# denyingmxd/CFPNet

Measured on AMD Instinct MI355X. Metric: depth maps/sec @ 480x640 bf16 (whole job; per_gpu = value / n_gpus); abs_rel vs CPU oracle, higher is better.
Workload: dtype bf16; 1 GPU; batch=8 480x640 RGB + 8x8-zone ToF, eval forward incl. the prob output [B,256,H/2,W/2] written in the storage dtype (bf16: 2 bytes/element); layers=hist2image combine1 image x2 (CFPNet), parallelism=single GPU

## Files before the change

### cfpnet_amd/csrc/conv_route.hip

```cpp
#include "conv_route.h"

namespace {

int tile_count(int variant, int M, int Cout) {
  static const int bm[4] = {256, 256, 128, 128}, bn[4] = {16, 32, 64, 128};
  return cdiv(M, bm[variant]) * cdiv(Cout, bn[variant]);
}

int pick_splits(int variant, int M, int Cout, int K, int dtype) {
  const int bk = is16(dtype) ? 32 : 16;
  const int nk = cdiv(K, bk);
  const int tiles = tile_count(variant, M, Cout);
  if (tiles >= 128 || nk < 16) return 1;
  int s = cdiv(256, tiles);
  if (s > nk / 6) s = nk / 6;
  if (s > 32) s = 32;
  return s < 2 ? 1 : s;
}

}

static int g_force_variant = -1, g_force_splits = -1;
int g_use_v1 = 0;
int g_tput = 0;
int g_probe = 0;
int g_x3_ad = 0;
int g_x3_small_m = 4800, g_x3_small_k = 1 << 30;
int g_x3_occ = 1;
static int x3_occ_of(int v) { return v == 13 ? 34 : v == 16 ? 35 : v == 15 ? 36 : v; }
static int x3_ad_of(int v) { return v == 26 ? 28 : v == 14 ? 29 : v == 13 ? 30 : v == 23 ? 31 : v == 16 ? 32 : v; }
int g_small_s2 = 1;
int g_up_halo = 1;
int g_halo_s2 = 1;
int g_halo = 1;
extern int g_bin_head_x3_rows;
int g_x3_ln_fused = 1;
int g_halo_x3 = 1;
static bool halo_x3_wins(long long M, int Cin, int Cout, bool tput) { return M >= (tput ? 30000 : 15000) && Cin <= 56; }
static int chunk_x3_variant(long long M, int Cin, int Cout, bool tput) {
  if (Cin % 32 != 0) return -1;
  if (Cin == 32) {
    if (Cout <= 32) return M >= 30000 ? 45 : -1;
    if (Cout > 64 && Cout <= 128 && !tput) return (M >= 30000 && M < 200000) ? 44 : -1;
    return -1;
  }
  if (Cout > 128) return (tput && M >= 9000) ? 36 : -1;
  if (Cout > 64) return M >= 30000 ? ((!tput && M < 200000) ? 44 : 36) : -1;
  if (Cout <= 32) return M >= (tput ? 30000 : 15000) ? 45 : -1;
  if (M >= 100000) return 38;
  if (M >= 30000) return tput ? 38 : 24;
  return -1;
}
int g_chunk16 = 1;
static int chunk16_variant(long long M, int Cin, int Cout, bool tput) {
  if (Cin <= 64 || Cin % 8 != 0 || Cout <= 0 || Cout % 8 != 0 || M <= 0 || g_chunk16 == 0) return -1;
  if (g_chunk16 == 2) return Cout > 64 ? 0 : 1;
  if (M >= 30000 && M < 200000) return 1;
  if (M >= 8000 && M < 12000) return (Cout > 128) != tput ? 1 : -1;
  return -1;
}
extern "C" int cfp_conv3x3_chunk_variant(int M, int Cin, int Cout, int in_flight) { return chunk16_variant(M, Cin, Cout, in_flight > 1); }
static bool halo_wins_s2(long long M, int Cout) { return g_halo == 2 || (g_halo == 1 && g_halo_s2 && M >= 30000 && Cout <= 160); }
static bool halo_wins(long long M, int Cout, bool tput) {
  if (g_halo == 2) return true;
  if (g_halo == 1 && tput && M >= 100000 && Cout <= 64) return true;
  return g_halo == 1 && ((M >= 300000 && (Cout <= 32 || Cout == 128)) || (M >= 100000 && Cout > 128 && Cout <= 160) ||
                         (M >= 30000 && Cout > 160 && Cout <= 256));
}
void cfp_tail_x3_debug_set(int value);
void cfp_fold_debug_set(int v);
void cfp_tail16_debug_set(int value);
void cfp_attn_apply_debug_set(int value);
void cfp_dwl3_debug_set(int value);
void cfp_dwl_wgrad_debug_set(int value);
void cfp_wgrad_debug_set(int value);
void cfp_bn_debug_set(int key, int value);
void cfp_attn_debug_set(int value);
int cfp_dw_debug_set(int key, int value);
extern "C" int cfp_debug_set(int key, int value) {
  switch (key) {
    case 3: case 4: case 5: case 6: case 9: case 10: case 11: return cfp_dw_debug_set(key, value);
    case 30: cfp_dwl3_debug_set(value); return CFP_OK;
    case 32: g_x3_occ = value; return CFP_OK;
    case 33: g_x3_small_m = value; return CFP_OK;
    case 34: g_x3_small_k = value; return CFP_OK;
    case 35: cfp_tail_x3_debug_set(value); return CFP_OK;
    case 37: cfp_fold_debug_set(value); return CFP_OK;
    case 38: cfp_attn_apply_debug_set(value); return CFP_OK;
    case 39: cfp_tail16_debug_set(value); return CFP_OK;
    case 40: g_chunk16 = value; return CFP_OK;
    case 17: g_tput = value; return CFP_OK;
    case 16: g_probe = (g_probe & 16) | value; return CFP_OK;
    case 29: g_x3_ad = value; return CFP_OK;
    case 28: g_probe = (g_probe & ~16) | (value ? 16 : 0); return CFP_OK;
    case 15: g_small_s2 = value; return CFP_OK;
    case 14: g_up_halo = value; return CFP_OK;
    case 19: cfp_attn_debug_set(value); return CFP_OK;
    case 20: case 21: cfp_bn_debug_set(key, value); return CFP_OK;
    case 22: cfp_wgrad_debug_set(value); return CFP_OK;
    case 23: cfp_dwl_wgrad_debug_set(value); return CFP_OK;
    case 18: g_halo_s2 = value; return CFP_OK;
    case 12: g_halo = value; return CFP_OK;
    case 24: g_halo_x3 = value; return CFP_OK;
    case 25: g_bin_head_x3_rows = value; return CFP_OK;
    case 26: g_x3_ln_fused = value; return CFP_OK;
    case 27: conv3x3_halo_debug_odd_pitch(value); return CFP_OK;
    case 13: conv3x3_halo_debug_stages(value); return CFP_OK;
    case 0: g_force_variant = value; return CFP_OK;
    case 1: g_force_splits = value; return CFP_OK;
    case 2: g_use_v1 = value; return CFP_OK;
    default: cfp_set_error("cfp_debug_set: unknown key"); return CFP_EINVAL;
  }
}

extern "C" int cfp_conv2d_variant(int M, int Cout) {
  if (Cout <= 16) return 0;
  if (Cout <= 32) return 1;
  if (Cout <= 64) return 2;
  long long t128 = (long long)cdiv(M, 128) * cdiv(Cout, 128);
  bool waste = (Cout % 128) != 0 && (Cout % 128) <= 64;
  return (t128 < 192 || waste) ? 2 : 3;
}

namespace {

struct Plan2 { int variant, splits; bool gen1; int direct; };

Plan2 plan2(long long M, int N, int K, int rpb, int B, bool allow_split, bool conv3x3s1 = false, bool tput = false) {
  Plan2 pl{4, 1, false, -1};
  const int nv = igemm2_num_variants();
  const bool big = M >= 100000, mid = M >= 30000;
  if (N <= 16) {
    if (big && K <= 144) pl.gen1 = true; else pl.variant = 16;
  } else if (N <= 32) {
    if (conv3x3s1 && K >= 576 && mid) pl.direct = 4;
    else if ((big && K <= 128) || (mid && K <= 64)) pl.gen1 = true;
    else pl.variant = mid ? 16 : 9;
  } else if (N <= 64) {
    if ((big && K <= 160) || (mid && K <= 64)) pl.gen1 = true;
    else pl.variant = big ? 14 : mid ? 13 : 4;
  } else {
    if ((big && K <= 288) || (mid && K <= 64)) pl.gen1 = true;
    else if ((M * N >= 614400ll * 128 && K >= 512) || (mid && K >= 2048)) pl.variant = 1;
    else if (mid) pl.variant = (N % 128 != 0 && N % 128 <= 64) ? 14 : 15;
    else if ((N >= 256 && K >= 2048) || N >= 1024) pl.variant = 12;
    else if (conv3x3s1 && N <= 128 && K >= 1152 && M >= 8000) pl.direct = 4;
    else pl.variant = 4;
  }
  if (rpb > 0) { pl.gen1 = false; pl.direct = -1; if (pl.variant != 12) pl.variant = 4; }
  if (pl.variant == 4 && !pl.gen1 && pl.direct < 0 && K >= 768) {
    const long long tm = rpb > 0 ? (long long)B * ((rpb + 63) / 64) : (M + 63) / 64;
    if (tm * ((N + 63) / 64) <= 256) pl.variant = 19;
  }
  if (allow_split && K >= 2048 && (M <= 1100 || ((M + 63) / 64) * ((N + 63) / 64) <= 48)) { pl.variant = 4; pl.splits = 8; pl.gen1 = false; pl.direct = -1; }
  if (pl.variant == 4 && pl.splits == 1 && !pl.gen1 && pl.direct < 0 && g_small_s2) pl.variant = 13;
  if (pl.variant == 12 && pl.splits == 1 && !pl.gen1 && pl.direct < 0 && g_small_s2) pl.variant = 15;
  if (pl.variant == 13 && !pl.gen1 && pl.direct < 0 && rpb == 0 && M >= 9000 && M < 30000 && N >= 512 && K <= 256 && g_small_s2) pl.variant = 14;
  if (!tput && !g_tput && conv3x3s1 && rpb == 0 && !pl.gen1 && pl.splits == 1 && pl.direct < 0 && M <= 2400 && N >= 256 && K >= 2048) pl.direct = 4;
  if ((tput || g_tput) && !pl.gen1 && pl.splits == 1) {
    if (pl.direct < 0 && M <= 20000 && N >= 256 && K >= 2048) pl.variant = 1;
    if (pl.direct < 0 && pl.variant == 13 && rpb == 0 && M >= 30000 && M < 100000 && N <= 64 && K >= 512) pl.variant = 14;
  }
  if (g_force_variant >= 200 && conv3x3s1 && g_force_variant - 200 < conv3x3_num_variants()) { pl.direct = g_force_variant - 200; pl.gen1 = false; pl.splits = 1; }
  else if (g_force_variant >= 0) pl.direct = -1;
  if (g_force_variant >= 0 && g_force_variant < nv) { pl.variant = g_force_variant; pl.gen1 = false; }
  if (g_force_splits >= 1) pl.splits = g_force_splits;
  if (pl.splits > 1 && pl.variant >= 19 && pl.variant <= 21 && g_force_variant < 0) pl.variant = 4;
  if (pl.direct >= 0) { pl.gen1 = false; pl.splits = 1; }
  return pl;
}

int pick_ln_variant(int Cout, long long M) {
  switch (Cout) {
    case 128: return M <= 20000 ? 12 : 1;
    case 64: return 2;
    case 32: return 8;
    case 16: return 11;
    default: return -1;
  }
}

}

static Plan2 plan_x3(long long M, int N, int K, int rpb, int B, bool allow_split, bool tput, bool piw_split = true) {
  Plan2 pl = plan2(M, N, 2 * (cdiv(K, 32) * 32), rpb, B, allow_split, false, tput);
  if (pl.gen1 || pl.direct >= 0) pl.variant = N <= 16 ? 10 : N <= 32 ? 16 : N <= 64 ? 14 : K <= 64 ? 16 : 1;
  pl.gen1 = false; pl.direct = -1;
  if (pl.variant == 0 || pl.variant == 1) pl.variant = 26;
  if (tput && pl.variant == 15 && M >= 9000 && N >= 128 && N <= 256 && K >= 500) pl.variant = 26;
  if (pl.variant < 0 || pl.variant >= igemm_x3_num_variants()) pl.variant = 13;
  if (!tput && rpb == 0 && pl.splits <= 1 && M <= 2400 && K >= 2000 && N >= 128 && (pl.variant == 15 || pl.variant == 13)) pl.variant = 19;
  if (!tput && rpb == 0 && allow_split && pl.splits <= 1 && K >= 2000 && (M <= 1200 || (M <= 4800 && K >= 2500))) {
    pl.variant = 13; pl.splits = (M <= 1200 && K >= 3000) ? 8 : 4;
  }
  if (!tput && rpb == 0 && pl.splits <= 1 && M <= 512 && N >= 512 && K <= 512) pl.variant = 17;
  if (!tput && pl.splits <= 1 && pl.variant == 13 && M <= g_x3_small_m && K <= g_x3_small_k) pl.variant = 17;
  if (!tput && rpb == 0 && pl.splits >= 4 && M <= 160 && (pl.variant == 4 || pl.variant == 13)) pl.variant = 17;
  if (rpb > 0 && !tput && piw_split && pl.splits <= 1) {
    const long long tiles = (long long)B * cdiv(rpb, 64) * cdiv(N, 64);
    const int nks = cdiv(K, 32);
    if (tiles <= 64 && nks >= 20) { pl.variant = 4; pl.splits = nks >= 40 ? 8 : 4; }
  }
  if (g_x3_ad && pl.splits <= 1) pl.variant = x3_ad_of(pl.variant);
  if (tput && g_x3_occ && pl.splits <= 1) pl.variant = x3_occ_of(pl.variant);
  return pl;
}

static ConvRoute route_x3(const ConvP& p, const ConvArgs& a) {
  ConvRoute r{};
  const bool tput = a.in_flight || g_tput != 0;
  const int rpb = a.per_image ? p.Ho * p.Wo : 0;
  const int chunk_v = g_halo_x3 ? chunk_x3_variant(p.M, p.Cin, p.Cout, tput) : -1;
  const bool halo = !a.per_image && !a.ln && conv3x3_halo_x3_takes(p) &&
                    (g_force_variant >= 500 || (g_force_variant < 0 && g_halo_x3 && (chunk_v >= 0 || halo_x3_wins(p.M, p.Cin, p.Cout, tput))));
  auto plan = [&](bool piw_split) { return plan_x3(p.M, p.Cout, p.K, rpb, p.B, rpb == 0, tput, piw_split); };
  Plan2 pl = plan(true);
  if (g_force_variant >= 400 && g_force_variant - 400 < igemm_x3_num_variants()) pl.variant = g_force_variant - 400;
  if (g_force_splits >= 1) pl.splits = g_force_splits;
  if (pl.splits > 1 && pl.variant >= 19) pl.variant = 4;
  if (pl.splits > 1 && a.ws_bytes < (size_t)pl.splits * p.M * p.Cout * sizeof(float) + (a.want_tickets ? CFP_CONV_TICKET_BYTES : 0)) {
    if (rpb > 0) pl = plan(false);
    pl.splits = 1;
  }
  int ln_v = -1;
  if (a.ln && rpb == 0 && g_x3_ln_fused) ln_v = p.Cout == 128 ? (p.M >= 30000 ? 26 : 27) : p.Cout == 64 ? (p.M >= 100000 ? 14 : 13) : p.Cout == 32 ? 16 : p.Cout == 16 ? 11 : -1;
  const int cv4 = p.Cout / 4;
  if (a.ln && pl.splits > 1 && p.Cout % 4 == 0 && cv4 <= 64 && (cv4 & (cv4 - 1)) == 0 && g_x3_ln_fused) {
    r.ln = ConvLn::Reduce;
  } else if (ln_v >= 0) {
    pl.variant = g_x3_ad ? x3_ad_of(ln_v) : ln_v; pl.splits = 1; r.ln = ConvLn::Tile;
  } else if (a.ln) {
    r.ln = ConvLn::After;
  }
  if (a.want_tickets && pl.splits > 1 && r.ln != ConvLn::Reduce) {
    int bm, bn, st;
    igemm_x3_variant_shape(pl.variant, &bm, &bn, &st);
    const long long tiles = (rpb > 0 ? (long long)p.B * cdiv(rpb, bm) : cdiv(p.M, bm)) * cdiv(p.Cout, bn);
    r.tickets = tiles <= CFP_TICKET_SLOTS && (long long)pl.splits * p.M * p.Cout * 4 < (1ll << 31) - 16;
  }
  r.fallback = {ConvFamily::X3, pl.variant};
  r.splits = pl.splits;
  r.first = r.fallback;
  if (halo) {
// ... 111 lines not shown
```

### cfpnet_amd/csrc/head_conv0.hip

```cpp
#include "common.h"

namespace {

typedef __attribute__((address_space(3))) void* lds_ptr_t;

constexpr int HC_C = 128;
constexpr int HC_NB = 256;
constexpr int HC_CIN = 32;
constexpr int HC_K0 = 9 * HC_CIN;
constexpr int HC_K3 = 9 * HC_C;
constexpr int HC_STEPS = HC_K3 / 64;
constexpr int HC_WSTAGE = HC_C * 128;
constexpr int HC_TW = 20, HC_TPIX = HC_TW * HC_TW, HC_TP = 80;
constexpr int HC_UW = 18, HC_UPIX = HC_UW * HC_UW, HC_UP = 288;
constexpr int HC_UGROUPS = (HC_UPIX + 15) / 16;
constexpr int HC_OFF_T = 2 * HC_WSTAGE;
constexpr int HC_OFF_U = 65536;
constexpr int HC_OFF_K = HC_OFF_U + HC_UPIX * HC_UP;
constexpr int HC_LDS = HC_OFF_K + 4 * 256 * 4;
constexpr int HC_BM = 256;
constexpr int HC_PPITCH = HC_BM + 8;
constexpr unsigned HC_OOB = 0x80000000u;
static_assert(HC_OFF_T + HC_TPIX * HC_TP <= HC_OFF_U, "t halo");
static_assert(HC_NB * HC_PPITCH * 2 <= HC_OFF_K, "prob staging must end before the constants");
static_assert(HC_LDS <= 160 * 1024, "LDS of a CU");

struct HeadC0P {
  const void* t; const void* w0; const float* scale0; const float* shift0;
  const void* w3; const float* scale3; const float* shift3;
  const void* wout; const float* bias_out; const float* centers;
  void* prob; float* pred;
  int t_ld, B, H, W, HW, tiles_x, tiles_y;
  int probe;
};

__device__ __forceinline__ void hc_handover() {
  asm volatile("s_waitcnt vmcnt(0) lgkmcnt(0)" ::: "memory");
  __syncthreads();
  asm volatile("" ::: "memory");
}

template <typename H>
__global__ __launch_bounds__(512, 1) void depth_head_conv0_kernel(HeadC0P p) {
  extern __shared__ __attribute__((aligned(16))) unsigned char smem[];
  unsigned char* sT = smem + HC_OFF_T;
  unsigned char* sU = smem + HC_OFF_U;
  float* sK = reinterpret_cast<float*>(smem + HC_OFF_K);
  const int tid = threadIdx.x;
  const int lane = tid & 63;
  const int wave = __builtin_amdgcn_readfirstlane(tid >> 6);
  const int fr = lane & 15, fq = lane >> 4;
  const int rsub = lane >> 3;
  const int lc = (lane & 7) ^ rsub;
  int bid = xcd_remap(blockIdx.x, gridDim.x);
  const int x0 = (bid % p.tiles_x) * 16; bid /= p.tiles_x;
  const int y0 = (bid % p.tiles_y) * 16;
  const int b = bid / p.tiles_y;

  const int live = (p.probe & 1) ? 0 : 1;
  const auto rs_t = __builtin_amdgcn_make_buffer_rsrc((void*)p.t, 0, (int)((unsigned)p.B * (unsigned)p.HW * (unsigned)p.t_ld * 2u) * live, 0x00020000);
  const auto rs_w0 = __builtin_amdgcn_make_buffer_rsrc((void*)p.w0, 0, HC_C * HC_K0 * 2 * live, 0x00020000);
  const auto rs_w3 = __builtin_amdgcn_make_buffer_rsrc((void*)p.w3, 0, HC_C * HC_K3 * 2 * live, 0x00020000);
  const auto rs_o = __builtin_amdgcn_make_buffer_rsrc((void*)p.wout, 0, HC_NB * HC_C * 2 * live, 0x00020000);

  auto issue_w0 = [&](int ks, int buf) {
#pragma unroll
    for (int i = 0; i < 2; ++i) {
      const int g = i * 8 + wave;
      const unsigned v = (ks * 8 + lc) * 8 < HC_K0 ? (unsigned)(g * 8 + rsub) * (unsigned)(HC_K0 * 2) + (unsigned)lc * 16u : HC_OOB;
      __builtin_amdgcn_raw_ptr_buffer_load_lds(rs_w0, (lds_ptr_t)(smem + buf * HC_WSTAGE + g * 1024), 16, (int)v, ks * 128, 0, 0);
    }
  };
  auto issue_w3 = [&](int ks, int buf) {
#pragma unroll
    for (int i = 0; i < 2; ++i) {
      const int g = i * 8 + wave;
      const unsigned v = (unsigned)(g * 8 + rsub) * (unsigned)(HC_K3 * 2) + (unsigned)lc * 16u;
      __builtin_amdgcn_raw_ptr_buffer_load_lds(rs_w3, (lds_ptr_t)(smem + buf * HC_WSTAGE + g * 1024), 16, (int)v, ks * 128, 0, 0);
    }
  };
  auto issue_wout = [&](int half, int off) {
#pragma unroll
    for (int q = 0; q < 4; ++q) {
      const int g = q * 8 + wave;
      const unsigned v = (unsigned)(g * 8 + rsub) * (unsigned)(HC_C * 2) + (unsigned)lc * 16u;
      __builtin_amdgcn_raw_ptr_buffer_load_lds(rs_o, (lds_ptr_t)(smem + off + g * 1024), 16, (int)v, half * 128, 0, 0);
    }
  };

  issue_w0(0, 0);

  {
    u32x4 v[4];
    int dst[4];
#pragma unroll
    for (int n = 0; n < 4; ++n) {
      const int i = tid + n * 512;
      const int px = i >> 2, ch = i & 3;
      const int hy = px / HC_TW, hx = px - hy * HC_TW;
      const int y = y0 - 2 + hy, x = x0 - 2 + hx;
      const bool ok = px < HC_TPIX && (unsigned)y < (unsigned)p.H && (unsigned)x < (unsigned)p.W;
      const unsigned off = ok ? (unsigned)((b * p.H + y) * p.W + x) * (unsigned)p.t_ld * 2u + (unsigned)ch * 16u : HC_OOB;
      v[n] = __builtin_amdgcn_raw_buffer_load_b128(rs_t, (int)off, 0, 0);
      dst[n] = px < HC_TPIX ? px * HC_TP + ch * 16 : -1;
    }
    if (tid < 256) {
      sK[tid] = p.bias_out[tid];
      sK[512 + tid] = p.centers[(long long)b * HC_NB + tid];
    } else if (tid < 384) {
      const int u = tid - 256;
      sK[256 + u] = p.scale3 ? p.scale3[u] : 1.f;
      sK[768 + u] = p.scale0 ? p.scale0[u] : 1.f;
    } else {
      const int u = tid - 384;
      sK[384 + u] = p.shift3 ? p.shift3[u] : 0.f;
      sK[896 + u] = p.shift0 ? p.shift0[u] : 0.f;
    }
#pragma unroll
    for (int n = 0; n < 4; ++n)
      if (dst[n] >= 0) *reinterpret_cast<u32x4*>(sT + dst[n]) = v[n];
  }

  {
    const int ng = wave + 16 < HC_UGROUPS ? 3 : 2;
    int tb[3];
#pragma unroll
    for (int g = 0; g < 3; ++g) {
      const int q = min((wave + 8 * g) * 16 + fr, HC_UPIX - 1);
      const int hy = q / HC_UW, hx = q - hy * HC_UW;
      tb[g] = (hy * HC_TW + hx) * HC_TP + fq * 16;
    }
    f32x4 acc0[3][8];
#pragma unroll
    for (int g = 0; g < 3; ++g)
#pragma unroll
      for (int i = 0; i < 8; ++i) acc0[g][i] = f32x4{0.f, 0.f, 0.f, 0.f};
#pragma unroll
    for (int ks = 0; ks < 5; ++ks) {
      hc_handover();
      if (ks < 4) issue_w0(ks + 1, (ks + 1) & 1);
      else issue_w3(0, 1);
      const unsigned char* cW = smem + (ks & 1) * HC_WSTAGE;
#pragma unroll
      for (int s = 0; s < 2; ++s) {
        const int tap = 2 * ks + s;
        if (tap >= 9) break;
        const int pc = ((s * 4 + fq) ^ (fr & 7)) * 16;
        const int toff = ((tap / 3) * HC_TW + tap % 3) * HC_TP;
        s16x8 wf[8], xf[3];
#pragma unroll
        for (int i = 0; i < 8; ++i) wf[i] = *reinterpret_cast<const s16x8*>(cW + (i * 16 + fr) * 128 + pc);
#pragma unroll
        for (int g = 0; g < 3; ++g)
          if (g < ng) xf[g] = *reinterpret_cast<const s16x8*>(sT + tb[g] + toff);
#pragma unroll
        for (int g = 0; g < 3; ++g)
          if (g < ng) {
#pragma unroll
            for (int i = 0; i < 8; ++i) acc0[g][i] = mfma16<H>(wf[i], xf[g], acc0[g][i]);
          }
      }
    }
#pragma unroll
    for (int g = 0; g < 3; ++g) {
      if (g >= ng) continue;
      const int q = (wave + 8 * g) * 16 + fr;
      const int hy = q / HC_UW, hx = q - hy * HC_UW;
      const int y = y0 - 1 + hy, x = x0 - 1 + hx;
      const bool inside = (unsigned)y < (unsigned)p.H && (unsigned)x < (unsigned)p.W;
#pragma unroll
      for (int i = 0; i < 8; ++i) {
        const int ch = i * 16 + fq * 4;
        float sc[4], sh[4], yv[4];
        Vec<float>::load(sK + 768 + ch, sc);
        Vec<float>::load(sK + 896 + ch, sh);
#pragma unroll
        for (int r = 0; r < 4; ++r) yv[r] = acc0[g][i][r] * sc[r] + sh[r];
        uint2 pk;
        pk.x = inside ? pack2<H>(yv[0], yv[1]) : 0u;
        pk.y = inside ? pack2<H>(yv[2], yv[3]) : 0u;
        if (q < HC_UPIX) *reinterpret_cast<uint2*>(sU + q * HC_UP + ch * 2) = pk;
      }
    }
  }
  if (p.probe & 8) {
    asm volatile("s_waitcnt vmcnt(0) lgkmcnt(0)" ::: "memory");
    return;
  }

  f32x4 acc1[8][2];
#pragma unroll
  for (int i = 0; i < 8; ++i)
#pragma unroll
    for (int j = 0; j < 2; ++j) acc1[i][j] = f32x4{0.f, 0.f, 0.f, 0.f};
  const unsigned char* urow = sU + ((2 * wave) * HC_UW + fr) * HC_UP + fq * 16;
  for (int ks = 0; ks < HC_STEPS; ++ks) {
    hc_handover();
    if (ks == 0) issue_wout(0, HC_OFF_T);
    if (ks + 1 < HC_STEPS) issue_w3(ks + 1, ks & 1);
    const int tap = ks >> 1;
    const int dy = tap / 3, dx = tap - dy * 3;
    const unsigned char* cP = urow + (dy * HC_UW + dx) * HC_UP + (ks & 1) * 128;
    const unsigned char* cW = smem + ((ks + 1) & 1) * HC_WSTAGE;
#pragma unroll
    for (int s = 0; s < 2; ++s) {
      const int pc = ((s * 4 + fq) ^ (fr & 7)) * 16;
      s16x8 wf[8], pf[2];
#pragma unroll
      for (int j = 0; j < 2; ++j) pf[j] = *reinterpret_cast<const s16x8*>(cP + j * (HC_UW * HC_UP) + s * 64);
#pragma unroll
      for (int i = 0; i < 8; ++i) wf[i] = *reinterpret_cast<const s16x8*>(cW + (i * 16 + fr) * 128 + pc);
#pragma unroll
      for (int i = 0; i < 8; ++i)
#pragma unroll
        for (int j = 0; j < 2; ++j) acc1[i][j] = mfma16<H>(wf[i], pf[j], acc1[i][j]);
    }
  }
  hc_handover();
  issue_wout(1, 0);
  if (p.probe & 2) {
    asm volatile("s_waitcnt vmcnt(0)" ::: "memory");
    if (tid == 0 && acc1[0][0][0] == 123.456f) p.pred[0] = acc1[7][1][3];
    return;
  }

  s16x8 bh[4][2];
#pragma unroll
  for (int kb = 0; kb < 4; ++kb) {
    float sc[2][4], sh[2][4];
#pragma unroll
    for (int u = 0; u < 2; ++u) {
      const int ch = (2 * kb + u) * 16 + fq * 4;
      Vec<float>::load(sK + 256 + ch, sc[u]);
      Vec<float>::load(sK + 384 + ch, sh[u]);
    }
#pragma unroll
    for (int j = 0; j < 2; ++j) {
      float v[8];
#pragma unroll
      for (int u = 0; u < 2; ++u)
#pragma unroll
        for (int r = 0; r < 4; ++r) v[u * 4 + r] = acc1[2 * kb + u][j][r] * sc[u][r] + sh[u][r];
      uint32_t hi[4];
#pragma unroll
      for (int e = 0; e < 4; ++e) {
        const H h0 = from_f32<H>(v[2 * e]), h1 = from_f32<H>(v[2 * e + 1]);
        hi[e] = (uint32_t)to_bits<H>(h0) | ((uint32_t)to_bits<H>(h1) << 16);
      }
      bh[kb][j] = __builtin_bit_cast(s16x8, u32x4{hi[0], hi[1], hi[2], hi[3]});
    }
  }

  __builtin_amdgcn_sched_barrier(0);

  f32x4 acc2[16][2];
#pragma unroll
  for (int ti = 0; ti < 16; ++ti) {
    float b4[4];
    Vec<float>::load(sK + ti * 16 + fq * 4, b4);
#pragma unroll
    for (int j = 0; j < 2; ++j) acc2[ti][j] = f32x4{b4[0], b4[1], b4[2], b4[3]};
  }
  auto gemm2_half = [&](int half, const unsigned char* base) {
#pragma unroll
    for (int kl = 0; kl < 2; ++kl) {
      const int kb = half * 2 + kl;
      const int pc = ((kl * 4 + fq) ^ (fr & 7)) * 16;
#pragma unroll
      for (int ti = 0; ti < 16; ++ti) {
        const s16x8 af = *reinterpret_cast<const s16x8*>(base + (ti * 16 + fr) * 128 + pc);
#pragma unroll
        for (int j = 0; j < 2; ++j) acc2[ti][j] = mfma16<H>(af, bh[kb][j], acc2[ti][j]);
      }
    }
  };
  gemm2_half(0, smem + HC_OFF_T);
  hc_handover();
  gemm2_half(1, smem);
  if (p.probe & 4) {
    if (tid == 0 && acc2[0][0][0] == 123.456f) p.pred[0] = acc2[15][1][3];
    return;
  }
  __syncthreads();

  H* sP = reinterpret_cast<H*>(smem);
  H* prob = reinterpret_cast<H*>(p.prob);
#pragma unroll
  for (int j = 0; j < 2; ++j) {
    const int pl = wave * 32 + j * 16 + fr;
    float mx = -3.0e38f;
#pragma unroll
    for (int ti = 0; ti < 16; ++ti)
#pragma unroll
      for (int r = 0; r < 4; ++r) mx = fmaxf(mx, acc2[ti][j][r]);
    mx = fmaxf(mx, __shfl_xor(mx, 16, 64));
    mx = fmaxf(mx, __shfl_xor(mx, 32, 64));
    float s = 0.f;
#pragma unroll
    for (int ti = 0; ti < 16; ++ti)
#pragma unroll
      for (int r = 0; r < 4; ++r) {
        const float d = acc2[ti][j][r] - mx;
        const float e = __expf(d);
        acc2[ti][j][r] = e;
        s += e;
      }
    s += __shfl_xor(s, 16, 64);
    s += __shfl_xor(s, 32, 64);
    const float inv = 1.f / s;
    float dot = 0.f;
#pragma unroll
    for (int ti = 0; ti < 16; ++ti) {
      float cen[4];
      Vec<float>::load(sK + 512 + ti * 16 + fq * 4, cen);
#pragma unroll
      for (int r = 0; r < 4; ++r) {
        const float pr = acc2[ti][j][r] * inv;
        dot = fmaf(pr, cen[r], dot);
        if (prob) sP[(ti * 16 + fq * 4 + r) * HC_PPITCH + pl] = from_f32<H>(pr);
      }
    }
    dot += __shfl_xor(dot, 16, 64);
    dot += __shfl_xor(dot, 32, 64);
    if (fq == 0) p.pred[(long long)b * p.HW + (y0 + 2 * wave + j) * p.W + x0 + fr] = dot;
  }
  if (!prob) return;
  __syncthreads();
#pragma unroll 4
  for (int q = tid; q < HC_NB * 32; q += 512) {
    const int n = q >> 5, c = q & 31;
    const int row = c >> 1, half = c & 1;
    *reinterpret_cast<u32x4*>(prob + ((long long)b * HC_NB + n) * p.HW + (y0 + row) * p.W + x0 + half * 8) =
        *reinterpret_cast<const u32x4*>(sP + n * HC_PPITCH + row * 16 + half * 8);
  }
}

}

extern "C" int cfp_depth_head_conv0_fused(const void* t, int t_ld, const void* w0, const float* scale0, const float* shift0, const void* w3,
                                          const float* scale3, const float* shift3, const void* wout_perm, const float* bias_out,
                                          const float* centers, void* prob, float* pred, int B, int H, int W, int flags, int dtype,
                                          cfp_stream_t stream) {
  CFP_REQUIRE(is16(dtype), CFP_EINVAL, "cfp_depth_head_conv0_fused: bf16/f16 only");
  CFP_REQUIRE(t && w0 && w3 && wout_perm && bias_out && centers && pred, CFP_EINVAL, "cfp_depth_head_conv0_fused: null pointer");
  CFP_REQUIRE(B > 0 && H > 0 && W > 0 && t_ld >= HC_CIN && t_ld % 8 == 0, CFP_ESHAPE, "cfp_depth_head_conv0_fused: bad shape (32 input channels, t_ld % 8 == 0)");
  CFP_REQUIRE(H % 16 == 0 && W % 16 == 0, CFP_ESHAPE, "cfp_depth_head_conv0_fused: H and W must be multiples of the 16 x 16 tile");
  const long long M = (long long)B * H * W;
  CFP_REQUIRE(M * t_ld * 2 < (1ll << 31) - 4096 && M / 256 < (1ll << 31), CFP_ESHAPE, "cfp_depth_head_conv0_fused: input larger than 2 GB");
  CFP_REQUIRE(aligned16(t) && aligned16(w0) && aligned16(w3) && aligned16(wout_perm) && aligned16(prob) && aligned16(bias_out) && aligned16(centers) &&
                  aligned16(scale0) && aligned16(shift0) && aligned16(scale3) && aligned16(shift3), CFP_EINVAL,
              "cfp_depth_head_conv0_fused: pointers must be 16-byte aligned");
  CFP_REQUIRE((flags & ~(15 << 8)) == 0, CFP_EINVAL, "cfp_depth_head_conv0_fused: unknown flags");
  static int lds_max = -1;
  if (lds_max < 0) {
    int dev = 0, v = 0;
    if (hipGetDevice(&dev) != hipSuccess || hipDeviceGetAttribute(&v, hipDeviceAttributeMaxSharedMemoryPerBlock, dev) != hipSuccess) {
      cfp_set_error("cfp_depth_head_conv0_fused: cannot query the LDS size");
      return CFP_EHIP;
    }
    lds_max = v;
  }
  CFP_REQUIRE(lds_max >= HC_LDS, CFP_ESHAPE, "cfp_depth_head_conv0_fused: the device does not grant 162944 bytes of LDS to a workgroup");
  HeadC0P p;
  p.t = t; p.w0 = w0; p.scale0 = scale0; p.shift0 = shift0; p.w3 = w3; p.scale3 = scale3; p.shift3 = shift3;
  p.wout = wout_perm; p.bias_out = bias_out; p.centers = centers; p.prob = prob; p.pred = pred;
  p.t_ld = t_ld; p.B = B; p.H = H; p.W = W; p.HW = H * W; p.tiles_x = W / 16; p.tiles_y = H / 16;
  p.probe = (flags >> 8) & 15;
  const int grid = (int)(M / HC_BM);
  hipStream_t s = reinterpret_cast<hipStream_t>(stream);
#define HC_LAUNCH(T)                                                                                                                       \
  do {                                                                                                                                     \
    static bool attr = false;                                                                                                              \
    if (!attr) {                                                                                                                           \
      if (hipFuncSetAttribute((const void*)depth_head_conv0_kernel<T>, hipFuncAttributeMaxDynamicSharedMemorySize, HC_LDS) != hipSuccess) { \
        cfp_set_error("cfp_depth_head_conv0_fused: cannot set the LDS size");                                                              \
        return CFP_EHIP;                                                                                                                   \
      }                                                                                                                                    \
      attr = true;                                                                                                                         \
    }                                                                                                                                      \
    hipLaunchKernelGGL((depth_head_conv0_kernel<T>), dim3(grid), dim3(512), HC_LDS, s, p);                                                 \
  } while (0)
  if (dtype == CFP_F16) HC_LAUNCH(f16_t);
  else HC_LAUNCH(bf16_t);
#undef HC_LAUNCH
  return cfp_check_launch("cfp_depth_head_conv0_fused");
}
```

### cfpnet_amd/ops.py

```python
from __future__ import annotations

import os
from dataclasses import dataclass
from typing import Optional, Tuple

import torch

from . import hip

DT = {torch.float32: hip.F32, torch.bfloat16: hip.BF16, torch.float16: hip.F16}


@dataclass
class Act:
    buf: torch.Tensor
    c0: int
    C: int

    @property
    def rows(self) -> int:
        return self.buf.shape[0]

    @property
    def ld(self) -> int:
# ... 384 lines not shown
        assert (drect if rec_side == 0 else srect) == ((0, 0, Hd, Wd) if rec_side == 0 else (0, 0, Hs, Ws)), "resize_bilinear(rec=): the fixed side is the whole map"
        hip.call("cfp_resize_bilinear_dev", src.ptr, src.ld, Hs, Ws, dst.ptr, dst.ld, Hd, Wd, _rec_ptr(rec), int(rec_side),
                 hip.ptr(zone_valid), zn, p1, p2, int(accumulate), B, src.C, src.dt, _s())
        return
    sy0, sx0, sh, sw = srect
    dy0, dx0, dh, dw = drect
    hip.call("cfp_resize_bilinear", src.ptr, src.ld, Hs, Ws, sy0, sx0, sh, sw, dst.ptr, dst.ld, Hd, Wd, dy0, dx0, dh, dw,
             hip.ptr(zone_valid), zn, p1, p2, int(accumulate), B, src.C, src.dt, _s())


def add_rowtable(x: Act, table, out: Act, rows, H, W, Wt, oy, ox):
    assert table.dtype == torch.float32 and table.shape[1] == x.C
    hip.call("cfp_add_rowtable", x.ptr, x.ld, table.data_ptr(), out.ptr, out.ld, rows, x.C, H, W, Wt, oy, ox, x.dt, _s())


def copy_rows(x: Act, out: Act, rows):
    hip.call("cfp_copy_rows", x.ptr, x.ld, out.ptr, out.ld, rows, x.C, x.dt, _s())


def upsample_cat_conv3x3(low: Act, Hs, Ws, skip: Act, w, scale, shift, out: Act, B, H, W, act, x3: bool = False):
    if x3:
        assert low.dt == skip.dt == out.dt == hip.F32 and w.dtype == torch.float16 and w.shape[-1] == 9 * (low.C + (skip.C + 31) // 32 * 32) * 2
        hip.call("cfp_upsample_cat_conv3x3", low.ptr, low.ld, Hs, Ws, low.C, skip.ptr, skip.ld, skip.C, w.data_ptr(),
                 hip.ptr(scale), hip.ptr(shift), out.ptr, out.ld, B, H, W, out.C, act, hip.F32X3, _s())
        return
    assert w.shape[-1] == 9 * (low.C + skip.C) and low.dt == skip.dt == out.dt
    hip.call("cfp_upsample_cat_conv3x3", low.ptr, low.ld, Hs, Ws, low.C, skip.ptr, skip.ld, skip.C, w.data_ptr(),
             hip.ptr(scale), hip.ptr(shift), out.ptr, out.ld, B, H, W, out.C, act, out.dt, _s())


def pack_w_x3_cat(w: torch.Tensor, cup: int) -> torch.Tensor:
    co, kh, kw, cin = w.shape
    assert kh == 3 and kw == 3 and cup % 32 == 0 and 0 < cup < cin
    csk = cin - cup
    pad = (csk + 31) // 32 * 32 - csk
    wp = torch.nn.functional.pad(w, (0, pad)) if pad else w
    return pack_w_x3(wp.reshape(co, 9 * (cup + csk + pad)).contiguous())


def copy_rows2(x0: Act, out0: Act, x1: Act, out1: Act, rows):
    assert x0.dt == x1.dt == out0.dt == out1.dt and out0.C == x0.C and out1.C == x1.C
    hip.call("cfp_copy_rows2", x0.ptr, x0.ld, out0.ptr, out0.ld, x0.C, x1.ptr, x1.ld, out1.ptr, out1.ld, x1.C, rows, x0.dt, _s())


def rgb_to_nhwc8(rgb: torch.Tensor, out: Act, B, H, W):
    assert rgb.dtype == torch.float32 and rgb.is_contiguous() and out.C == 8 and out.ld == 8
    hip.call("cfp_rgb_to_nhwc8", rgb.data_ptr(), out.ptr, B, H, W, out.dt, _s())


def rgb_to_nhwc8_hilo(rgb: torch.Tensor, out: Act, B, H, W):
    assert rgb.dtype == torch.float32 and rgb.is_contiguous() and out.C == 8 and out.ld == 8
    hip.call("cfp_rgb_to_nhwc8_hilo", rgb.data_ptr(), out.ptr, B, H, W, out.dt, _s())


def scalar_to_rows8(x: torch.Tensor, out: Act, rows):
    assert x.dtype == torch.float32 and x.is_contiguous() and out.C == 8 and out.ld == 8
    hip.call("cfp_scalar_to_rows8", x.data_ptr(), out.ptr, rows, out.dt, _s())


def bin_regressor(partial, nsplit, inv_hw, w1x1, w0, b0, w1, b1, w2, b2, min_val, max_val, norm, edges, centers, B, C,
                  hidden, nbins):
    hip.call("cfp_bin_regressor", partial.data_ptr(), nsplit, float(inv_hw), w1x1.data_ptr(), w0.data_ptr(), b0.data_ptr(),
             w1.data_ptr(), b1.data_ptr(), w2.data_ptr(), b2.data_ptr(), float(min_val), float(max_val), norm,
             edges.data_ptr(), centers.data_ptr(), B, C, hidden, nbins, _s())


def _check_stats(stats, B, HW):
    assert stats.dtype == torch.float32 and stats.is_contiguous() and stats.numel() == B * 3 * HW, "stats: float32 [B, 3, HW]"


def bin_softmax(logits: Act, centers, prob, pred, B, HW, nbins, stats=None):
    if stats is None:
        hip.call("cfp_bin_softmax", logits.ptr, logits.ld, centers.data_ptr(), hip.ptr(prob), pred.data_ptr(), B, HW, nbins,
                 logits.dt, _s())
        return
    _check_stats(stats, B, HW)
    hip.call("cfp_bin_softmax_stats", logits.ptr, logits.ld, centers.data_ptr(), hip.ptr(prob), pred.data_ptr(), stats.data_ptr(), B, HW,
             nbins, logits.dt, _s())


def bin_head_fused(x: Act, w, bias, centers, prob, pred, B, HW, stats=None):
    x3 = x.buf.dtype == torch.float32 and w.dtype == torch.float16
    assert not x3 or (tuple(w.shape) == (256, (x.C + 31) // 32 * 64) and (prob is None or prob.dtype == torch.float32))
    if stats is None:
        hip.call("cfp_bin_head_fused", x.ptr, x.ld, w.data_ptr(), bias.data_ptr(), centers.data_ptr(), hip.ptr(prob),
                 pred.data_ptr(), B, HW, x.C, hip.F32X3 if x3 else x.dt, _s())
        return
    _check_stats(stats, B, HW)
    hip.call("cfp_bin_head_fused_stats", x.ptr, x.ld, w.data_ptr(), bias.data_ptr(), centers.data_ptr(), hip.ptr(prob),
             pred.data_ptr(), stats.data_ptr(), B, HW, x.C, hip.F32X3 if x3 else x.dt, _s())


def permute_wout(w: torch.Tensor, dtype, hilo: bool = True, diffuse: bool = False) -> torch.Tensor:
    w = w.detach().float().reshape(w.shape[0], -1)
    assert w.shape == (256, 128)
    src = pw_k_order(128)
    wp = w[:, src]
    hi = (round_taps(w.reshape(256, 1, 128), dtype).reshape(256, 128)[:, src] if diffuse else wp).to(dtype)
    planes = [hi]
    if hilo:
        planes.append((wp - hi.float()).to(dtype))
    return torch.stack(planes).contiguous()


def pw_k_order(K: int) -> torch.Tensor:
    pos = torch.arange((K + 31) // 32 * 32)
    kb, q, e = pos // 32, (pos % 32) // 8, pos % 8
    src = 32 * kb + 16 * (e // 4) + 4 * q + (e % 4)
    return torch.where(src < K, src, torch.full_like(src, -1))


def pad_pw_w(w: torch.Tensor) -> torch.Tensor:
    co, K = w.shape
    out = torch.zeros((co + 15) // 16 * 16, (K + 31) // 32 * 32, dtype=w.dtype, device=w.device)
    out[:co, :K] = w
    return out.contiguous()


def conv3x3_pw_fused_variant(Cin: int, Cmid: int, Cout: int, stride: int, dt: int) -> int:
    return int(hip.load().cfp_conv3x3_pw_fused_variant(Cin, Cmid, Cout, stride, dt))


def conv3x3_pw_fused(x: Act, w1: torch.Tensor, s1, t1, act1, w2_pad: torch.Tensor, s2, t2, out: Act, B, H, W, stride, pad_t, pad_l, Ho, Wo,
                     act2=hip.ACT_NONE, residual: Optional[Act] = None):
    mid = w1.shape[0]
    assert x.rows >= B * H * W and out.rows >= B * Ho * Wo and x.dt == out.dt
    assert w1.dtype == x.buf.dtype and tuple(w1.shape) == (mid, 9 * x.C) and w1.is_contiguous()
    assert w2_pad.dtype == x.buf.dtype and tuple(w2_pad.shape) == ((out.C + 15) // 16 * 16, (mid + 31) // 32 * 32) and w2_pad.is_contiguous()
    hip.call("cfp_conv3x3_pw_fused", x.ptr, x.ld, w1.data_ptr(), hip.ptr(s1), hip.ptr(t1), act1, w2_pad.data_ptr(), hip.ptr(s2), hip.ptr(t2), act2,
             residual.ptr if residual else 0, residual.ld if residual else 0, out.ptr, out.ld, B, H, W, x.C, mid, out.C, stride, pad_t, pad_l,
             Ho, Wo, x.dt, _s())


def depth_head_fused(x: Act, w3, scale3, shift3, wout_perm: torch.Tensor, bias_out, centers, prob, pred, B, H, W, ram_out: Optional[Act] = None,
                     ram_hilo: bool = True, probe: int = 0, stats=None):
    assert x.C == 128 and w3.shape == (128, 9 * 128) and wout_perm.shape[1:] == (256, 128) and wout_perm.dtype == x.buf.dtype
    flags = (hip.HEAD_WOUT_HILO if wout_perm.shape[0] == 2 else 0) | (hip.HEAD_RAM_HILO if ram_hilo else 0) | (probe << 8)
    if ram_out is not None:
        assert ram_out.ld == 128 and ram_out.C == 128
    if stats is None:
        hip.call("cfp_depth_head_fused", x.ptr, x.ld, w3.data_ptr(), hip.ptr(scale3), hip.ptr(shift3), wout_perm.data_ptr(), bias_out.data_ptr(),
                 centers.data_ptr(), hip.ptr(prob), pred.data_ptr(), ram_out.ptr if ram_out is not None else 0, B, H, W, flags, x.dt, _s())
        return
    _check_stats(stats, B, H * W)
    hip.call("cfp_depth_head_fused_stats", x.ptr, x.ld, w3.data_ptr(), hip.ptr(scale3), hip.ptr(shift3), wout_perm.data_ptr(), bias_out.data_ptr(),
             centers.data_ptr(), hip.ptr(prob), pred.data_ptr(), stats.data_ptr(), ram_out.ptr if ram_out is not None else 0, B, H, W, flags,
             x.dt, _s())


def depth_head_conv0_fits(H: int, W: int) -> bool:
    return H % 16 == 0 and W % 16 == 0


def depth_head_conv0_fused(t: Act, w0, scale0, shift0, w3, scale3, shift3, wout_perm: torch.Tensor, bias_out, centers, prob, pred, B, H, W,
                           probe: int = 0):
    assert t.C == 32 and t.rows >= B * H * W and tuple(w0.shape) == (128, 9 * 32) and tuple(w3.shape) == (128, 9 * 128)
    assert tuple(wout_perm.shape) == (1, 256, 128) and wout_perm.dtype == t.buf.dtype and w0.dtype == t.buf.dtype and w3.dtype == t.buf.dtype
    hip.call("cfp_depth_head_conv0_fused", t.ptr, t.ld, w0.data_ptr(), hip.ptr(scale0), hip.ptr(shift0), w3.data_ptr(), hip.ptr(scale3),
             hip.ptr(shift3), wout_perm.data_ptr(), bias_out.data_ptr(), centers.data_ptr(), hip.ptr(prob), pred.data_ptr(), B, H, W,
             probe << 8, t.dt, _s())


def hist_encoder(hist: torch.Tensor, blob: torch.Tensor, layout, outs, R: int, pe=(None, None, None), n_pe: int = 0):
    import ctypes
    assert hist.dtype == torch.float32 and hist.is_contiguous() and hist.numel() >= R and blob.dtype == torch.float32 and len(layout) == 9
    flat = [int(v) for row in layout for v in row]
    arr = (ctypes.c_int * len(flat))(*flat)
    for o, row in zip(outs, layout[2::3]):
        assert o.C == row[4] and o.ld == o.C and o.c0 == 0 and o.rows >= R
    for t, o in zip(pe, outs):
        assert t is None or (t.dtype == torch.float32 and tuple(t.shape) == (n_pe, o.C) and t.is_contiguous())
    hip.call("cfp_hist_encoder", hist.data_ptr(), blob.data_ptr(), ctypes.addressof(arr), outs[0].ptr, outs[1].ptr, outs[2].ptr,
             hip.ptr(pe[0]), hip.ptr(pe[1]), hip.ptr(pe[2]), n_pe, R, outs[0].dt, _s())


def conv3x3_mean(partial: torch.Tensor, nsplit, x: Act, w32: torch.Tensor, bias, msum: torch.Tensor, B, H, W, Cout):
    assert w32.dtype == torch.float32 and tuple(w32.shape) == (Cout, 9 * x.C) and msum.dtype == torch.float32 and msum.numel() >= B * Cout
    hip.call("cfp_conv3x3_mean", partial.data_ptr(), nsplit, x.ptr, x.ld, w32.data_ptr(), hip.ptr(bias), msum.data_ptr(), B, H, W, x.C, Cout, x.dt, _s())


def mbconv_plan(B, H, W, Cin, mid):
    import ctypes
    t, kp = ctypes.c_int(0), ctypes.c_int(0)
    rc = hip.load().cfp_mbconv_plan(B, H, W, Cin, mid, ctypes.byref(t), ctypes.byref(kp))
    return (t.value, kp.value) if rc == 0 else None


def pack_mbconv_pw(w2d: torch.Tensor, dtype) -> torch.Tensor:
    mid, cin = w2d.shape
    kp = (cin + 31) // 32 * 32
    out = torch.zeros(mid, kp + 8, dtype=dtype)
    out[:, :cin] = w2d.to(dtype)
    return out.contiguous()


def mbconv_expand_dw(x: Act, wpw: torch.Tensor, s1, t1, wdw: torch.Tensor, s2, t2, out: Act, partial: Optional[torch.Tensor], B, H, W):
    mid = out.C
    assert wpw.dtype == x.buf.dtype and wpw.shape[0] == mid and wdw.shape == (9, mid) and wdw.dtype == x.buf.dtype
    hip.call("cfp_mbconv_expand_dw", x.ptr, x.ld, wpw.data_ptr(), s1.data_ptr(), t1.data_ptr(), wdw.data_ptr(), s2.data_ptr(), t2.data_ptr(),
             out.ptr, out.ld, hip.ptr(partial), B, H, W, x.C, mid, x.dt, _s())


def lkpm_tail(t: Act, xin: Act, out: Act, w1, b1, w2, b2, ln_g, ln_b, rows, ln_eps=1e-6):
    D = t.C
    x3 = t.buf.dtype == torch.float32 and w1.dtype == torch.float16
    k1, k2 = (2 * D, 8 * D) if x3 else (D, 4 * D)
    assert xin.C == D and out.C == D and tuple(w1.shape) == (4 * D, k1) and tuple(w2.shape) == (D, k2) and (x3 or w1.dtype == t.buf.dtype)
    hip.call("cfp_lkpm_tail", t.ptr, t.ld, xin.ptr, xin.ld, out.ptr, out.ld, w1.data_ptr(), b1.data_ptr(), w2.data_ptr(), b2.data_ptr(),
             ln_g.data_ptr(), ln_b.data_ptr(), float(ln_eps), rows, D, hip.F32X3 if x3 else t.dt, _s())
```

Baseline: 4068 maps/s.

## Compute head softmax tail in registers with DPP-packed prob stores

The fused depth-head kernel gains a register-resident softmax/expectation tail. It reduces max and sum with cross-lane shuffles and packs bf16 probabilities via DPP swizzles into 16-byte stores straight to global memory. This skips the LDS staging pass and its barrier. A second template option adds software-pipelined MFMA loops with sched_group_barrier interleaving, but the defaults (tail=1, loops=2) select only the register tail with the original loops. The risk is higher register pressure and less coalesced prob stores than the LDS-transposed path.

Measured after the change: 4099 maps/s (median of 6 runs). About the same (+0.8%).

```diff
diff --git a/cfpnet_amd/csrc/conv_route.hip b/cfpnet_amd/csrc/conv_route.hip
--- a/cfpnet_amd/csrc/conv_route.hip
+++ b/cfpnet_amd/csrc/conv_route.hip
@@ -76,6 +76,7 @@
 void cfp_wgrad_debug_set(int value);
 void cfp_bn_debug_set(int key, int value);
 void cfp_attn_debug_set(int value);
+int cfp_head_conv0_debug_set(int key, int value);
 int cfp_dw_debug_set(int key, int value);
 extern "C" int cfp_debug_set(int key, int value) {
   switch (key) {
@@ -89,6 +90,7 @@
     case 38: cfp_attn_apply_debug_set(value); return CFP_OK;
     case 39: cfp_tail16_debug_set(value); return CFP_OK;
     case 40: g_chunk16 = value; return CFP_OK;
+    case 41: case 42: return cfp_head_conv0_debug_set(key, value);
     case 17: g_tput = value; return CFP_OK;
     case 16: g_probe = (g_probe & 16) | value; return CFP_OK;
     case 29: g_x3_ad = value; return CFP_OK;
diff --git a/cfpnet_amd/csrc/head_conv0.hip b/cfpnet_amd/csrc/head_conv0.hip
--- a/cfpnet_amd/csrc/head_conv0.hip
+++ b/cfpnet_amd/csrc/head_conv0.hip
@@ -1,4 +1,5 @@
 #include "common.h"
+#include <type_traits>
 
 namespace {
 
@@ -40,7 +41,14 @@
   asm volatile("" ::: "memory");
 }
 
-template <typename H>
+__device__ __forceinline__ uint32_t hc_quad_xor1(uint32_t v) { return (uint32_t)__builtin_amdgcn_mov_dpp((int)v, 0xB1, 0xf, 0xf, true); }
+__device__ __forceinline__ uint32_t hc_quad_xor2(uint32_t v) { return (uint32_t)__builtin_amdgcn_mov_dpp((int)v, 0x4E, 0xf, 0xf, true); }
+__device__ __forceinline__ uint32_t hc_row_xor4(uint32_t v) {
+  const int up = __builtin_amdgcn_update_dpp(0, (int)v, 0x104, 0xf, 0x5, false);
+  return (uint32_t)__builtin_amdgcn_update_dpp(up, (int)v, 0x114, 0xf, 0xa, false);
+}
+
+template <typename H, int TAIL, int PIPE>
 __global__ __launch_bounds__(512, 1) void depth_head_conv0_kernel(HeadC0P p) {
   extern __shared__ __attribute__((aligned(16))) unsigned char smem[];
   unsigned char* sT = smem + HC_OFF_T;
@@ -141,6 +149,41 @@
       if (ks < 4) issue_w0(ks + 1, (ks + 1) & 1);
       else issue_w3(0, 1);
       const unsigned char* cW = smem + (ks & 1) * HC_WSTAGE;
+      if constexpr (PIPE) {
+        const int nt = ks < 4 ? 2 : 1;
+        s16x8 wf[2][8], xf[2][3];
+#pragma unroll
+        for (int s = 0; s < nt; ++s) {
+          const int tap = 2 * ks + s;
+          const int pc = ((s * 4 + fq) ^ (fr & 7)) * 16;
+          const int toff = ((tap / 3) * HC_TW + tap % 3) * HC_TP;
+#pragma unroll
+          for (int g = 0; g < 3; ++g) xf[s][g] = *reinterpret_cast<const s16x8*>(sT + tb[g] + toff);
+#pragma unroll
+          for (int i = 0; i < 8; ++i) wf[s][i] = *reinterpret_cast<const s16x8*>(cW + (i * 16 + fr) * 128 + pc);
+        }
+#pragma unroll
+        for (int s = 0; s < nt; ++s)
+#pragma unroll
+          for (int g = 0; g < 2; ++g)
+#pragma unroll
+            for (int i = 0; i < 8; ++i) acc0[g][i] = mfma16<H>(wf[s][i], xf[s][g], acc0[g][i]);
+        if (nt == 2) {
+          __builtin_amdgcn_sched_group_barrier(0x100, 11, 0);
+#pragma unroll
+          for (int q = 0; q < 11; ++q) {
+            __builtin_amdgcn_sched_group_barrier(0x008, 1, 0);
+            __builtin_amdgcn_sched_group_barrier(0x100, 1, 0);
+          }
+        }
+        if (ng == 3) {
+#pragma unroll
+          for (int s = 0; s < nt; ++s)
+#pragma unroll
+            for (int i = 0; i < 8; ++i) acc0[2][i] = mfma16<H>(wf[s][i], xf[s][2], acc0[2][i]);
+        }
+        continue;
+      }
 #pragma unroll
       for (int s = 0; s < 2; ++s) {
         const int tap = 2 * ks + s;
@@ -202,6 +245,31 @@
     const int dy = tap / 3, dx = tap - dy * 3;
     const unsigned char* cP = urow + (dy * HC_UW + dx) * HC_UP + (ks & 1) * 128;
     const unsigned char* cW = smem + ((ks + 1) & 1) * HC_WSTAGE;
+    if constexpr (PIPE) {
+      s16x8 wf[2][8], pf[2][2];
+#pragma unroll
+      for (int s = 0; s < 2; ++s) {
+        const int pc = ((s * 4 + fq) ^ (fr & 7)) * 16;
+#pragma unroll
+        for (int j = 0; j < 2; ++j) pf[s][j] = *reinterpret_cast<const s16x8*>(cP + j * (HC_UW * HC_UP) + s * 64);
+#pragma unroll
+        for (int i = 0; i < 8; ++i) wf[s][i] = *reinterpret_cast<const s16x8*>(cW + (i * 16 + fr) * 128 + pc);
+      }
+#pragma unroll
+      for (int s = 0; s < 2; ++s)
+#pragma unroll
+        for (int i = 0; i < 8; ++i)
+#pragma unroll
+          for (int j = 0; j < 2; ++j) acc1[i][j] = mfma16<H>(wf[s][i], pf[s][j], acc1[i][j]);
+      __builtin_amdgcn_sched_group_barrier(0x100, 10, 0);
+#pragma unroll
+      for (int q = 0; q < 10; ++q) {
+        __builtin_amdgcn_sched_group_barrier(0x008, 1, 0);
+        __builtin_amdgcn_sched_group_barrier(0x100, 1, 0);
+      }
+      __builtin_amdgcn_sched_group_barrier(0x008, 22, 0);
+      continue;
+    }
 #pragma unroll
     for (int s = 0; s < 2; ++s) {
       const int pc = ((s * 4 + fq) ^ (fr & 7)) * 16;
@@ -262,6 +330,28 @@
     for (int j = 0; j < 2; ++j) acc2[ti][j] = f32x4{b4[0], b4[1], b4[2], b4[3]};
   }
   auto gemm2_half = [&](int half, const unsigned char* base) {
+    if constexpr (PIPE) {
+      s16x8 af[32];
+      __builtin_amdgcn_sched_barrier(0);
+#pragma unroll
+      for (int q = 0; q < 32; ++q) {
+        const int kl = q >> 4, ti = q & 15;
+        af[q] = *reinterpret_cast<const s16x8*>(base + (ti * 16 + fr) * 128 + ((kl * 4 + fq) ^ (fr & 7)) * 16);
+      }
+#pragma unroll
+      for (int q = 0; q < 32; ++q)
+#pragma unroll
+        for (int j = 0; j < 2; ++j) acc2[q & 15][j] = mfma16<H>(af[q], bh[half * 2 + (q >> 4)][j], acc2[q & 15][j]);
+      __builtin_amdgcn_sched_group_barrier(0x100, 4, 0);
+#pragma unroll
+      for (int q = 0; q < 28; ++q) {
+        __builtin_amdgcn_sched_group_barrier(0x008, 2, 0);
+        __builtin_amdgcn_sched_group_barrier(0x100, 1, 0);
+      }
+      __builtin_amdgcn_sched_group_barrier(0x008, 8, 0);
+      __builtin_amdgcn_sched_barrier(0);
+      return;
+    }
 #pragma unroll
     for (int kl = 0; kl < 2; ++kl) {
       const int kb = half * 2 + kl;
@@ -281,10 +371,77 @@
     if (tid == 0 && acc2[0][0][0] == 123.456f) p.pred[0] = acc2[15][1][3];
     return;
   }
+  H* prob = reinterpret_cast<H*>(p.prob);
+  if constexpr (TAIL) {
+    auto tail = [&](auto with_prob) {
+      constexpr bool WP = decltype(with_prob)::value;
+      const uint32_t sel = (fr & 1) ? 0x03020706u : 0x05040100u;
+      const bool upper = (fr & 2) != 0;
+#pragma unroll
+      for (int j = 0; j < 2; ++j) {
+        float mx = -3.0e38f;
+#pragma unroll
+        for (int ti = 0; ti < 16; ++ti)
+#pragma unroll
+          for (int r = 0; r < 4; ++r) mx = fmaxf(mx, acc2[ti][j][r]);
+        mx = fmaxf(mx, __shfl_xor(mx, 16, 64));
+        mx = fmaxf(mx, __shfl_xor(mx, 32, 64));
+        float s = 0.f;
+#pragma unroll
+        for (int ti = 0; ti < 16; ++ti)
+#pragma unroll
+          for (int r = 0; r < 4; ++r) {
+            const float d = acc2[ti][j][r] - mx;
+            const float e = __expf(d);
+            acc2[ti][j][r] = e;
+            s += e;
+          }
+        s += __shfl_xor(s, 16, 64);
+        s += __shfl_xor(s, 32, 64);
+        const float inv = 1.f / s;
+        float dot = 0.f;
+        H* pl = nullptr;
+        uint2 held = {0u, 0u};
+        if constexpr (WP) pl = prob + ((long long)b * HC_NB + fq * 4 + (fr & 3)) * p.HW + (y0 + 2 * wave + j) * p.W + x0 + (fr & 12);
+#pragma unroll
+        for (int ti = 0; ti < 16; ++ti) {
+          float cen[4], pr[4];
+          Vec<float>::load(sK + 512 + ti * 16 + fq * 4, cen);
+#pragma unroll
+          for (int r = 0; r < 4; ++r) {
+            pr[r] = acc2[ti][j][r] * inv;
+            dot = fmaf(pr[r], cen[r], dot);
+          }
+          if constexpr (WP) {
+            const uint32_t p01 = pack2<H>(pr[0], pr[1]), p23 = pack2<H>(pr[2], pr[3]);
+            const uint32_t y0w = __builtin_amdgcn_perm(hc_quad_xor1(p01), p01, sel);
+            const uint32_t y1w = __builtin_amdgcn_perm(hc_quad_xor1(p23), p23, sel);
+            const uint32_t z0 = hc_quad_xor2(y0w), z1 = hc_quad_xor2(y1w);
+            uint2 o;
+            o.x = upper ? z1 : y0w;
+            o.y = upper ? y1w : z0;
+            if ((ti & 1) == 0) {
+              held = o;
+            } else {
+              const bool oddq = (fr & 4) != 0;
+              const uint32_t gx = hc_row_xor4(oddq ? held.x : o.x), gy = hc_row_xor4(oddq ? held.y : o.y);
+              const u32x4 w = oddq ? u32x4{gx, gy, o.x, o.y} : u32x4{held.x, held.y, gx, gy};
+              *reinterpret_cast<u32x4*>(pl + (long long)(ti - 1) * 16 * p.HW + (oddq ? (long long)16 * p.HW - 4 : 0)) = w;
+            }
+          }
+        }
+        dot += __shfl_xor(dot, 16, 64);
+        dot += __shfl_xor(dot, 32, 64);
+        if (fq == 0) p.pred[(long long)b * p.HW + (y0 + 2 * wave + j) * p.W + x0 + fr] = dot;
+      }
+    };
+    if (prob) tail(std::true_type{});
+    else tail(std::false_type{});
+    return;
+  }
   __syncthreads();
 
   H* sP = reinterpret_cast<H*>(smem);
-  H* prob = reinterpret_cast<H*>(p.prob);
 #pragma unroll
   for (int j = 0; j < 2; ++j) {
     const int pl = wave * 32 + j * 16 + fr;
@@ -335,6 +492,39 @@
   }
 }
 
+int g_hc_tail = 0;
+int g_hc_loops = 0;
+constexpr int HC_TAIL_DEFAULT = 1, HC_LOOPS_DEFAULT = 2;
+
+template <typename H, int TAIL, int PIPE>
+int hc_launch(const HeadC0P& p, int grid, hipStream_t s) {
+  static bool attr = false;
+  if (!attr) {
+    if (hipFuncSetAttribute((const void*)depth_head_conv0_kernel<H, TAIL, PIPE>, hipFuncAttributeMaxDynamicSharedMemorySize, HC_LDS) != hipSuccess) {
+      cfp_set_error("cfp_depth_head_conv0_fused: cannot set the LDS size");
+      return CFP_EHIP;
+    }
+    attr = true;
+  }
+  hipLaunchKernelGGL((depth_head_conv0_kernel<H, TAIL, PIPE>), dim3(grid), dim3(512), HC_LDS, s, p);
+  return CFP_OK;
+}
+template <typename H>
+int hc_launch_form(const HeadC0P& p, int grid, hipStream_t s) {
+  const bool regs = (g_hc_tail ? g_hc_tail : HC_TAIL_DEFAULT) == 1, pipe = (g_hc_loops ? g_hc_loops : HC_LOOPS_DEFAULT) == 1;
+  if (regs) return pipe ? hc_launch<H, 1, 1>(p, grid, s) : hc_launch<H, 1, 0>(p, grid, s);
+  return pipe ? hc_launch<H, 0, 1>(p, grid, s) : hc_launch<H, 0, 0>(p, grid, s);
+}
+
+}
+
+int cfp_head_conv0_debug_set(int key, int value) {
+  if (value < 0 || value > 2) {
+    cfp_set_error("cfp_debug_set: keys 41 / 42 take 0 (default), 1 (new form) or 2 (earlier form)");
+    return CFP_EINVAL;
+  }
+  (key == 41 ? g_hc_tail : g_hc_loops) = value;
+  return CFP_OK;
 }
 
 extern "C" int cfp_depth_head_conv0_fused(const void* t, int t_ld, const void* w0, const float* scale0, const float* shift0, const void* w3,
@@ -368,20 +558,7 @@
   p.probe = (flags >> 8) & 15;
   const int grid = (int)(M / HC_BM);
   hipStream_t s = reinterpret_cast<hipStream_t>(stream);
-#define HC_LAUNCH(T)                                                                                                                       \
-  do {                                                                                                                                     \
-    static bool attr = false;                                                                                                              \
-    if (!attr) {                                                                                                                           \
-      if (hipFuncSetAttribute((const void*)depth_head_conv0_kernel<T>, hipFuncAttributeMaxDynamicSharedMemorySize, HC_LDS) != hipSuccess) { \
-        cfp_set_error("cfp_depth_head_conv0_fused: cannot set the LDS size");                                                              \
-        return CFP_EHIP;                                                                                                                   \
-      }                                                                                                                                    \
-      attr = true;                                                                                                                         \
-    }                                                                                                                                      \
-    hipLaunchKernelGGL((depth_head_conv0_kernel<T>), dim3(grid), dim3(512), HC_LDS, s, p);                                                 \
-  } while (0)
-  if (dtype == CFP_F16) HC_LAUNCH(f16_t);
-  else HC_LAUNCH(bf16_t);
-#undef HC_LAUNCH
+  const int rc = dtype == CFP_F16 ? hc_launch_form<f16_t>(p, grid, s) : hc_launch_form<bf16_t>(p, grid, s);
+  if (rc != CFP_OK) return rc;
   return cfp_check_launch("cfp_depth_head_conv0_fused");
 }
diff --git a/cfpnet_amd/ops.py b/cfpnet_amd/ops.py
--- a/cfpnet_amd/ops.py
+++ b/cfpnet_amd/ops.py
@@ -560,10 +560,17 @@
     return H % 16 == 0 and W % 16 == 0
 
 
+def depth_head_conv0_forms(tail: int = 0, loops: int = 0):
+    hip.call("cfp_debug_set", 41, int(tail))
+    hip.call("cfp_debug_set", 42, int(loops))
+
+
 def depth_head_conv0_fused(t: Act, w0, scale0, shift0, w3, scale3, shift3, wout_perm: torch.Tensor, bias_out, centers, prob, pred, B, H, W,
-                           probe: int = 0):
+                           probe: int = 0, forms=None):
     assert t.C == 32 and t.rows >= B * H * W and tuple(w0.shape) == (128, 9 * 32) and tuple(w3.shape) == (128, 9 * 128)
     assert tuple(wout_perm.shape) == (1, 256, 128) and wout_perm.dtype == t.buf.dtype and w0.dtype == t.buf.dtype and w3.dtype == t.buf.dtype
+    if forms is not None:
+        depth_head_conv0_forms(*forms)
     hip.call("cfp_depth_head_conv0_fused", t.ptr, t.ld, w0.data_ptr(), hip.ptr(scale0), hip.ptr(shift0), w3.data_ptr(), hip.ptr(scale3),
              hip.ptr(shift3), wout_perm.data_ptr(), bias_out.data_ptr(), centers.data_ptr(), hip.ptr(prob), pred.data_ptr(), B, H, W,
              probe << 8, t.dt, _s())
```
